# dguilliams3/book-recommendation-engine

Measured on AMD Instinct MI355X. Metric: exact top-10 queries/sec at 10M×1536 fp32 (1/8 GPU) + % HBM/MFMA roofline, higher is better.
Workload: dtype fp32

## Files before the change

book-recommendation-engine_amd/csrc/vs_api.hip:

```cpp
#include <algorithm>
#include <cstdio>
#include <cstring>
#include <mutex>
#include <shared_mutex>
#include <string>
#include <vector>

#include "../../include/vsearch.h"
#include "vs_internal.h"

using namespace vs;

constexpr int kI8FirstBackoff = 8;
constexpr int kI8MaxBackoff = 64;

struct vs_index {
  int d = 0;
  int metric = VS_METRIC_L2;
  int dtype = VS_DTYPE_F32;
  int device = 0;
  int esize = 4;
  int64_t ld = 0;
  int64_t ntotal = 0;
  int64_t capacity = 0;
// ... 652 lines not shown
    idx->rn2[p] = nullptr;
  }
  if (idx->fscale) (void)hipFree(idx->fscale);
  if (idx->anorm) (void)hipFree(idx->anorm);
  if (idx->anorm_b) (void)hipFree(idx->anorm_b);
  idx->anorm_b = nullptr;
  idx->codes = nullptr;
  idx->norms = nullptr;
  idx->fscale = nullptr;
  idx->anorm = nullptr;
  idx->capacity = 0;
}

struct SearchArgs {
  int mode = MODE_IP;
  const float* qbuf = nullptr;
  const void* qb16 = nullptr;
  const float* qaux = nullptr;
  const float* xaux = nullptr;
  int nq = 0, nq_pad = 0, k = 0;
  int64_t self0 = -1;
  float min_score = 0.0f;
  int raw = 0;
  bool l2_direct = false;
  bool host_wait = false;
  float* D = nullptr;
  int64_t* I = nullptr;
};

int run_topk(vs_index* idx, const SearchArgs& a, hipStream_t st, int force_engine);

int run_gemm(vs_index* idx, const SearchArgs& a, int need, hipStream_t st,
              const int* qlist = nullptr, const int* qcount = nullptr) {
  const int KP = kp_for(need);
  const int ntotal = (int)idx->ntotal;
  Scratch scr(st);
  Partials part;
  part.KP = KP;
  const int nqt = a.nq_pad / kBQ;
  const int ntiles = (ntotal + kBN - 1) / kBN;
  const int nsplit = qlist ? (int)std::max<int64_t>(1, std::min<int64_t>(ntiles, 256))
                           : (int)std::max<int64_t>(1, std::min<int64_t>(ntiles, (512 + nqt - 1) / nqt));
  part.P = 2 * nsplit;
  const size_t n = (size_t)a.nq_pad * part.P * KP;
  VS_HIP(scr.alloc((void**)&part.key, n * sizeof(float)), "vs: scratch");
  VS_HIP(scr.alloc((void**)&part.id, n * sizeof(int)), "vs: scratch");
  const void* qmat = a.qb16 ? a.qb16 : (const void*)a.qbuf;
  {
    KernelTimer tm(st, qlist ? nullptr : "gemm_topk");
    VS_HIP(launch_gemm_topk(KP, a.mode, idx->codes, a.xaux, qmat, a.qaux, idx->ld, idx->esize,
                            ntotal, a.nq_pad, nsplit, a.self0, part, st, qlist, qcount),
           "vs: gemm_topk launch");
    tm.stop();
  }
  VS_HIP(launch_merge_partials(a.mode, part, qlist ? a.nq_pad : a.nq, a.k, idx->id_base,
                               a.min_score, a.D, a.I, a.k, st, a.raw, qlist, qcount),
         "vs: merge launch");
  return VS_OK;
}

int adaptive_record(vs_index* idx, const int* handed, int n, hipStream_t st);
int run_paged(vs_index* idx, const SearchArgs& a, hipStream_t st, const int* gl = nullptr,
              const int* gc = nullptr);
int run_gemm_rescored(vs_index* idx, const SearchArgs& a, int need, int KF, int plane,
                      hipStream_t st, const int* gl, const int* gc);

static bool dump_enabled() {
  static const bool v = [] {
    const char* e = getenv("VS_X1_DUMP");
    return !e || atoi(e) != 0;
  }();
  return v;
}

static bool dump_mfma32() {
  const char* e = getenv("VS_X1_DUMP_MFMA");
  return e && atoi(e) == 32;
}

static int recut_mode() {
  const char* e = getenv("VS_X1_RECUT");
  const int v = e ? atoi(e) : 1;
  return v == 0 ? 0 : v == 2 ? 2 : 1;
}

constexpr int64_t kSmallFilterMinRows = 1 << 18;
bool small_filter_on() {
  const char* e = getenv("VS_SMALL_FILTER");
  return !e || atoi(e) != 0;
}
bool small_l2d_ok(int mode, const SearchArgs& a) {
  if (!(mode == MODE_L2 && a.l2_direct)) return true;
  const char* e = getenv("VS_SMALL_L2D");
  return !e || atoi(e) != 0;
}

bool skinny_deep_on() {
  const char* e = getenv("VS_SKINNY_DEEP");
  return !e || atoi(e) != 0;
}

static int x1_wg_target(int nqt) {
  const char* e = getenv("VS_X1_WGS");
  const int v = e ? atoi(e) : 0;
  return v > 0 ? v : nqt <= 8 ? 256 : 512;
}

static bool tail_wait_on(const SearchArgs& a, hipStream_t st) {
  const char* e = getenv("VS_TAIL_WAIT");
  if (e && atoi(e) == 0) return false;
  if (a.host_wait) return true;
  hipStreamCaptureStatus cs = hipStreamCaptureStatusNone;
  if (hipStreamIsCapturing(st, &cs) != hipSuccess) {
    (void)hipGetLastError();
    return false;
  }
  return cs == hipStreamCaptureStatusNone;
}

static int read_count(const int* dcount, hipStream_t st, int* out) {
  static thread_local int* pin = nullptr;
  if (!pin) VS_HIP(hipHostMalloc((void**)&pin, sizeof(int), hipHostMallocPortable), "vs: count");
  VS_HIP(hipMemcpyAsync(pin, dcount, sizeof(int), hipMemcpyDeviceToHost, st), "vs: count");
  VS_HIP(hipStreamSynchronize(st), "vs: count");
  *out = *pin;
  return VS_OK;
}

int run_filter_verify(vs_index* idx, const SearchArgs& a, int need, int KF, hipStream_t st,
                      int plane, bool last_plane, bool deep = false, const int* gl = nullptr,
                      const int* gc = nullptr) {
  const int ntotal = (int)idx->ntotal;
  const int mode = a.mode;
  const bool gathered = gl != nullptr;
  Scratch scr(st);
  X1Args x;
  x.nq_pad = (int)round_up(a.nq_pad, kX1Q);
  const int nq = gathered ? x.nq_pad : a.nq;
  const int nqt = x.nq_pad / kX1Q;
  const int ntiles = (ntotal + kX1Q - 1) / kX1Q;
  const int L = x1_lane_len();
  const int lists_per_cand = mode == MODE_IP && KF >= 64 ? 8 : 4;
  const int wg_target = x1_wg_target(nqt);
  x.nsplit = (int)std::max<int64_t>(
      std::min<int64_t>(ntiles, lists_per_cand * ((KF + L - 1) / L)),
      std::min<int64_t>(ntiles, (wg_target + nqt - 1) / nqt));
  if (deep)
    x.nsplit = (int)std::max<int64_t>(
        x.nsplit, std::min<int64_t>({ntiles, 512, (1ll << 30) / ((int64_t)x.nq_pad * 4 * 8 * 8)}));
  if (!gathered && !deep && plane == FILTER_BF16)
    x.nsplit = (int)std::min<int64_t>(ntiles, 2 * (int64_t)x.nsplit);
  const bool small = !gathered && !deep && a.nq <= skinny_plane_max_queries() && a.self0 < 0 &&
                     (mode == MODE_IP || (mode == MODE_L2 && idx->l2aug()));
  if (small) x.nsplit = (int)std::min<int64_t>(512, std::max<int64_t>(1, (ntiles + 3) / 4));
  x.nsplit = std::max(x.nsplit, 1);
  {
    static const int mult = [] {
      const char* e = getenv("VS_X1_SPLIT_MULT");
      return e && atoi(e) > 1 ? atoi(e) : 1;
    }();
    x.nsplit = (int)std::min<int64_t>(ntiles, (int64_t)x.nsplit * mult);
  }
  Partials part;
  part.KP = L;
  part.P = 4 * x.nsplit;
  const size_t np_ = (size_t)x.nq_pad * part.P * part.KP;
// ... 37 lines not shown
    if (i8) {
      float *sc = nullptr, *r = nullptr;
      VS_HIP(scr.alloc((void**)&sc, (size_t)qa_rows * sizeof(float)), "vs: scratch");
      VS_HIP(scr.alloc((void**)&r, (size_t)qa_rows * sizeof(float)), "vs: scratch");
      if (aug)
        VS_HIP(launch_quantize_i8_l2aug(Q, idx->ld, 0, qa_rows, idx->aug, nullptr, (int8_t*)qh, sc,
                                        r, nullptr, st),
               "vs: query plane");
      else
        VS_HIP(launch_quantize_i8(Q, idx->ld, 0, qa_rows, (int8_t*)qh, sc, r, st),
               "vs: query plane");
      qs = sc;
      qr2 = r;
    } else if (aug) {
      VS_HIP(launch_bf16_plane_l2aug(Q, idx->ld, 0, qa_rows, idx->aug, nullptr, (uint16_t*)qh,
                                     nullptr, nullptr, st),
             "vs: query plane");
    } else {
      VS_HIP(launch_bf16_plane(Q, idx->ld, 0, qa_rows, (uint16_t*)qh, st), "vs: query plane");
    }
    VS_HIP(launch_plane_zero_rows(qh, pb, qa_rows, x.nq_pad - qa_rows, st), "vs: query plane");
    QH = qh;
  }
  const unsigned* stats = idx->bstats[plane];
  x.filter = plane;
  x.XH = idx->fplane[plane];
  x.xs = idx->fscale;
  if (i8 && mode == MODE_COS) {
    float* cx = nullptr;
    VS_HIP(scr.alloc((void**)&cx, (size_t)idx->capacity * sizeof(float)), "vs: scratch");
    VS_HIP(launch_mul_arrays(idx->fscale, a.xaux, idx->capacity, cx, st), "vs: cosine factors");
    x.xs = cx;
    if (plane_rows) {
      qs = cx + a.self0;
    } else {
      float* cq = nullptr;
      VS_HIP(scr.alloc((void**)&cq, (size_t)qa_rows * sizeof(float)), "vs: scratch");
      VS_HIP(launch_mul_arrays(qs, qaux, qa_rows, cq, st), "vs: cosine factors");
      qs = cq;
    }
  }
  if (i8) {
    float* gm = nullptr;
    const size_t ng = (size_t)(idx->capacity / 16);
    VS_HIP(scr.alloc((void**)&gm, 2 * ng * sizeof(float)), "vs: scratch");
    VS_HIP(launch_group_max(x.xs, idx->capacity, gm, st, ntotal, gm + ng), "vs: factor bounds");
    x.xgmax = gm;
    x.xgmin = gm + ng;
  }
  x.xaux = a.xaux;
  x.QH = QH;
  x.qs = qs;
  x.qaux = qaux;
  x.nqa = qa_rows;
  x.ld = !aug ? idx->ld : i8 ? idx->ld + idx->aug_m : idx->ld + kAugBf16;
  x.ntotal = ntotal;
  x.self0 = self_rows ? a.self0 : -1;
  x.qrow = qrow;
  x.qcount = gc;
  const BoundArgs ba = aug ? make_bound_args_l2aug(idx->ld, idx->aug, plane)
                           : make_bound_args(idx->ld, plane);
  if (!gathered && !small && x1_dump_applies(kmode, plane) && dump_enabled() &&
      x1_pass_dumps(ntotal, x.nsplit)) {
    const int64_t lists = (int64_t)x.nq_pad * part.P;
    const int dR = (int)std::min<int64_t>(x1_dump_slots(), (int64_t(4) << 30) / (lists * 8));
    if (dR >= 16) {
      int *dc = nullptr, *ds = nullptr;
      hipError_t e = scr.alloc((void**)&dc, (size_t)lists * sizeof(int));
      if (e == hipSuccess) e = scr.alloc((void**)&ds, (size_t)lists * dR * 2 * sizeof(int));
      if (e == hipSuccess) {
        VS_HIP(scr.alloc((void**)&x.qcut, (size_t)qa_rows * sizeof(float)), "vs: scratch");
        double* bk = nullptr;
        VS_HIP(scr.alloc((void**)&bk, (size_t)qa_rows * sizeof(double)), "vs: scratch");
        VS_HIP(hipMemsetD32Async((hipDeviceptr_t)x.qcut, 0x7f7fffff, (size_t)qa_rows, st),
               "vs: cuts");
        VS_HIP(hipMemsetAsync(dc, 0, (size_t)lists * sizeof(int), st), "vs: dumps");
        VS_HIP(launch_qbound(mode, Q, idx->ld, qaux, plane, stats, qr2, qa_rows, bk, st, &ba),
               "vs: cuts");
        x.qbkey = bk;
        x.qcut_m = need;
        x.dump = true;
        x.dump32 = dump_mfma32();
        x.recut = recut_mode();
        x.dcount = dc;
        x.dslot = ds;
        x.dR = dR;
        x.dstats = device_stats(idx->device) ? device_stats(idx->device) + 6 : nullptr;
      } else {
        (void)hipGetLastError();
      }
    }
  }
  {
    KernelTimer whole(st, gathered ? nullptr : i8 ? "gemm_topk_x1_i8_pass" : "gemm_topk_x1_pass",
                      false);
    X1SpanTimer tm(i8 ? "gemm_topk_x1_i8" : "gemm_topk_x1",
                   i8 ? "gemm_topk_x1_i8_list" : "gemm_topk_x1_list");
    if (!gathered) x.timing = &tm;
    if (gathered && deep && !i8 && kmode == MODE_IP && a.self0 < 0 && skinny_deep_on()) {
      VS_HIP(launch_skinny_plane(FILTER_BF16, x.XH, x.QH, x.ld, ntotal, gc, nullptr, nullptr, part,
                                 st),
             "vs: skinny deep stage");
      x.qskip = skinny_plane_max_queries();
    }
    if (small) {
      int* cnt = nullptr;
      VS_HIP(scr.alloc((void**)&cnt, sizeof(int)), "vs: scratch");
      VS_HIP(hipMemsetD32Async((hipDeviceptr_t)cnt, a.nq, 1, st), "vs: count");
      KernelTimer ks(st, i8 ? "skinny_plane_topk_i8" : "skinny_plane_topk");
      VS_HIP(launch_skinny_plane(plane, x.XH, x.QH, x.ld, ntotal, cnt, qs, x.xs, part, st, a.nq),
             "vs: skinny first stage");
      ks.stop();
    } else {
      int nd = 0;
      VS_HIP(launch_gemm_topk_x1(kmode, x, part, st, &nd), "vs: gemm_topk_x1 launch");
    }
    x.timing = nullptr;
    whole.stop();
  }
  if (aug)
    VS_HIP(launch_l2aug_map(part.key, part.id, (int64_t)part.P * part.KP, qa_rows, qaux,
                            idx->aug.nref, x.qcut, st),
           "vs: L2 keys");

  float* Dk = nullptr;
  int64_t* Ik = nullptr;
  VS_HIP(scr.alloc((void**)&Dk, (size_t)nq * KF * sizeof(float)), "vs: scratch");
  VS_HIP(scr.alloc((void**)&Ik, (size_t)nq * KF * sizeof(int64_t)), "vs: scratch");
  if (KF > 64) {
    VS_HIP(launch_select_lists(part, L, nq, KF, Dk, Ik, st, gc), "vs: merge");
  } else if (select_heads_applies(part, L, KF)) {
    VS_HIP(launch_select_heads(part, nq, KF, Dk, Ik, st, gc), "vs: merge");
  } else {
    Partials mp = part;
    mp.KP = kp_for(KF);
    mp.KL = L;
    VS_HIP(launch_merge_partials(MODE_L2, mp, nq, KF, 0, 0.0f, Dk, Ik, KF, st, 0, nullptr, gc),
           "vs: merge");
  }
  Partials vp;
  vp.KP = kp_for(KF);
  vp.P = 1;
  int* flags = nullptr;
  int* qlist = nullptr;
  int* qcount = nullptr;
  VS_HIP(scr.alloc((void**)&vp.key, (size_t)nq * vp.KP * sizeof(float)), "vs: scratch");
  VS_HIP(scr.alloc((void**)&vp.id, (size_t)nq * vp.KP * sizeof(int)), "vs: scratch");
  VS_HIP(scr.alloc((void**)&flags, (size_t)nq * sizeof(int)), "vs: scratch");
  VS_HIP(scr.alloc((void**)&qlist, (size_t)x.nq_pad * sizeof(int)), "vs: scratch");
  VS_HIP(scr.alloc((void**)&qcount, 2 * sizeof(int)), "vs: scratch");
  const float* qinv = mode == MODE_COS ? qaux : nullptr;
  const float* xinv = mode == MODE_COS ? a.xaux : nullptr;
  VS_HIP(launch_verify_rescore(vmode, nq, KF, need, Dk, Ik, idx->codes, idx->norms, Q, qaux,
                               idx->ld, ba, stats, part, L, vp.key, vp.id, vp.KP, flags, st, qinv,
                               xinv, qr2, gc, x.qcut, idx->esize),
         "vs: verify");
  unsigned long long* dst = device_stats(idx->device);
  if (!dst) return fail(VS_E_HIP, "vs: statistics buffer");
  VS_HIP(launch_compact_flags(flags, nq, qlist, qcount, dst + 1, gathered ? nullptr : dst + 0, st),
         "vs: flags");
  if (wide_enabled())
    VS_HIP(launch_verify_wide(vmode, nq, qlist, qcount, KF, need, idx->codes, idx->norms, Q, qaux,
                              idx->ld, ba, stats, part, L, vp.key, vp.id, vp.KP, flags, st, qinv,
                              xinv, qr2, Dk, Ik, dst + 4, x.qcut, idx->esize),
           "vs: verify wide");
  VS_HIP(launch_compact_flags(flags, nq, qlist, qcount + 1, last_plane ? dst + 2 : dst + 3,
// ... 1306 lines not shown
```

book-recommendation-engine_amd/csrc/vs_gemm_x1.hip:

```cpp
#include <algorithm>
#include <climits>
#include <cmath>
#include <cstdlib>
#include <type_traits>

#include "vs_device.h"

#ifndef VS_X1_PROBE
#define VS_X1_PROBE 0
#endif
#define VS_X1_P(bit) ((VS_X1_PROBE & (bit)) != 0)

namespace vs {

#ifndef VS_X1_STAMP
#define VS_X1_STAMP 0
#endif
constexpr int kStampSeg = 9;
constexpr int kStampCnt = 3;
constexpr int kStampN = 2 * (kStampSeg + kStampCnt) + 2;
__device__ unsigned long long g_x1_stamps[kStampN];

namespace {

// ... 996 lines not shown
        pkey[o + e] = FLT_MAX;
        pid[o + e] = -1;
      }
    }
  }
}

template <int KR, int EL>
__global__ __launch_bounds__(256) void x1_replay_kernel(
    int* __restrict__ dcount, const int* __restrict__ dslot, float* __restrict__ pkey,
    int* __restrict__ pid, int P, int KP, int nqa, const float* __restrict__ qs,
    const float* __restrict__ xs, int64_t self0, int ntotal, int dR, int64_t nl,
    float* __restrict__ qcut, unsigned long long* __restrict__ stats) {
  const int64_t i = (int64_t)blockIdx.x * 256 + threadIdx.x;
  const int cnt = i < (int64_t)nqa * P ? dcount[i] : 0;
  {
    unsigned long long a = (unsigned long long)cnt, b = cnt > dR ? 1ull : 0ull;
    for (int o = 32; o > 0; o >>= 1) {
      a += __shfl_xor(a, o);
      b += __shfl_xor(b, o);
    }
    if ((threadIdx.x & 63) == 0 && a && stats) {
      atomicAdd(stats, a);
      if (b) atomicAdd(stats + 1, b);
    }
  }
  if (cnt == 0) return;
  dcount[i] = 0;
  const int q = (int)(i / P);
  if (cnt > dR) {
    qcut[q] = -FLT_MAX;
    return;
  }
  const float cut = qcut[q];
  const float qsc = EL == FILTER_I8 ? qs[q] : 0.0f;
  const int selfrow = self0 >= 0 ? (int)(self0 + q) : -1;
  static_assert(KR % 4 == 0, "lane lists move as 16-B pieces");
  float lk[KR];
  int li[KR];
  const int64_t o = i * KP;
#pragma unroll
  for (int e = 0; e < KR; e += 4) {
    const f32x4 kv = *(const f32x4*)(pkey + o + e);
    const int4 iv = *(const int4*)(pid + o + e);
    lk[e] = kv.x, lk[e + 1] = kv.y, lk[e + 2] = kv.z, lk[e + 3] = kv.w;
    li[e] = iv.x, li[e + 1] = iv.y, li[e + 2] = iv.z, li[e + 3] = iv.w;
  }
  const i32x2* sl = (const i32x2*)dslot + i;
  constexpr int kB = 8;
  for (int c0 = 0; c0 < cnt; c0 += kB) {
    i32x2 e[kB];
    float fx[kB];
#pragma unroll
    for (int j = 0; j < kB; ++j) e[j] = c0 + j < cnt ? sl[(int64_t)(c0 + j) * nl] : i32x2{-1, 0};
#pragma unroll
    for (int j = 0; j < kB; ++j)
      fx[j] = EL == FILTER_I8 && e[j][0] >= 0 && e[j][0] < ntotal ? xs[e[j][0]] : 0.0f;
#pragma unroll
    for (int j = 0; j < kB; ++j) {
      const int row = e[j][0];
      if (!(row >= 0 && row < ntotal && row != selfrow)) continue;
      const float key = x1_key<EL>(e[j][1], qsc, fx[j]);
      if (key < fminf(lk[KR - 1], cut)) list_insert<KR, int>(lk, li, key, row);
    }
  }
#pragma unroll
  for (int e = 0; e < KR; e += 4) {
    *(f32x4*)(pkey + o + e) = f32x4{lk[e], lk[e + 1], lk[e + 2], lk[e + 3]};
    *(int4*)(pid + o + e) = make_int4(li[e], li[e + 1], li[e + 2], li[e + 3]);
  }
}

static int x1_qg() {
  static const int v = [] {
    const char* e = getenv("VS_X1_QG");
    const int q = e ? atoi(e) : 0;
    return q > 0 ? q : 4;
  }();
  return v;
}

static hipError_t launch_qcut(const X1Args& a, Partials part, hipStream_t st);
static hipError_t launch_x1_replay_cut(const X1Args& a, Partials part, hipStream_t st);

static bool x1_group_rounds() {
  const char* e = getenv("VS_X1_XCDG");
  return !e || atoi(e) != 0;
}

constexpr int kHybMinTiles = 16;
constexpr int kX1SplitDen = 8;
static bool x1_hybrid_on() {
  const char* e = getenv("VS_X1_HYB");
  return e && atoi(e) != 0;
}

constexpr int kX1ShortChunkTiles = 40;
static int x1_chunk_tiles(int per_block, bool can_dump) {
  const char* e = getenv("VS_X1_CHUNK_TILES");
  const int v = e ? atoi(e) : 0;
  if (v > 0) return v;
  return can_dump && per_block >= 128 && per_block <= 3 * kX1ChunkTiles ? kX1ShortChunkTiles
                                                                        : kX1ChunkTiles;
}

static int x1_split_den() {
  const char* e = getenv("VS_X1_SPLIT");
  return e ? std::max(0, atoi(e)) : kX1SplitDen;
}
static bool x1_split_segments(int den) {
  const char* e = getenv("VS_X1_SPLITSEG");
  return e && atoi(e) != 0 && den >= 4 && (den & (den - 1)) == 0;
}
constexpr int kSplitMinTiles = 16;
static int x1_first_den(int el) {
  const char* e = getenv("VS_X1_QUARTER");
  if (!e) return el == FILTER_BF16 ? 4 : 0;
  const int v = atoi(e);
  return v == 1 ? 4 : v >= 2 ? v : 0;
}

template <int KR, int MODE, int EL>
static hipError_t x1_launch(const X1Args& a, Partials part, hipStream_t st, int* ndispatch) {
  const int ntiles = (a.ntotal + kT - 1) / kT;
  const int nqt = a.nq_pad / kT;
  const int per_block = (ntiles + a.nsplit - 1) / a.nsplit;
  const int qg = a.qcount ? nqt : x1_qg() * (x1_group_rounds() ? 1 : -1);
  const bool dump = a.dump && x1_has_dump(MODE, EL) && !a.qcount && a.qcut && a.qbkey &&
                    a.qcut_m > 0 && a.dcount && a.dslot && a.dR > 0;
  const int chunk_tiles = x1_chunk_tiles(per_block, dump);
  int nchunk = a.qcount ? 1 : std::max(1, (per_block + chunk_tiles - 1) / chunk_tiles);
  const int den = x1_split_den();
  const bool split = dump && nchunk < 4 && den >= 2 && per_block >= kSplitMinTiles;
  const bool cutting = dump && (nchunk >= 4 || split);
  const int tiles0 = (per_block + nchunk - 1) / nchunk;
  const bool hyb = dump && !split && x1_hybrid_on() && tiles0 >= kHybMinTiles;
  const bool later_dump = cutting || hyb;
  const int F = x1_first_den(EL);
  const bool quarter = cutting && !split && nchunk >= 4 && F >= 2 && per_block / (F * nchunk) >= 2;
  const bool sseg = split && x1_split_segments(den);
  int lg = 0;
  while ((1 << lg) < den) ++lg;
  const int nparts = split ? den : quarter ? F * nchunk : nchunk;
  const int nlaunch = sseg ? lg + 1 : split ? 2 : quarter ? nchunk + 1 : nchunk;
  const int64_t ldb = a.ld * filter_bytes(EL);
  if (a.qtile0 < 0) return hipErrorInvalidValue;
  for (int c = 0; c < nlaunch; ++c) {
    const int p0 = sseg    ? (c == 0 ? 0 : 1 << (c - 1))
                   : split   ? (c == 0 ? 0 : 1)
                   : quarter ? (c == 0 ? 0 : c == 1 ? 1 : F * (c - 1))
                             : c;
    const int p1 = sseg    ? (c == 0 ? 1 : 1 << c)
                   : split   ? (c == 0 ? 1 : den)
                   : quarter ? (c == 0 ? 1 : F * c)
                             : c + 1;
    if (a.timing)
      a.timing->begin(st, !(later_dump && nlaunch > 1) || c > 0, (double)(p1 - p0) / nparts);
    if (later_dump && c > 0 && x1_has_s16(MODE, EL) && !a.dump32) {
      if constexpr (x1_has_s16(MODE, EL))
        hipLaunchKernelGGL((gemm_topk_x1<KR, MODE, true, EL, false, true>), dim3(nqt * a.nsplit),
                           dim3(512), 0, st, (const char*)a.XH, a.xs, a.xaux, (const char*)a.QH,
                           a.qs, a.qaux, a.nqa, (int)(ldb / 64), a.ntotal, ntiles, a.nsplit, nqt,
                           a.qtile0, a.self0, a.qrow, a.qcount, p0, p1, nparts, part.KP, qg,
                           part.key, part.id, a.xgmax, a.xgmin, a.qcut, a.dcount, a.dslot, a.dR,
                           a.qskip);
    } else if (later_dump && c > 0) {
      if constexpr (x1_has_dump(MODE, EL))
        hipLaunchKernelGGL((gemm_topk_x1<KR, MODE, true, EL>), dim3(nqt * a.nsplit), dim3(512), 0,
                           st, (const char*)a.XH, a.xs, a.xaux, (const char*)a.QH, a.qs, a.qaux,
                           a.nqa, (int)(ldb / 64), a.ntotal, ntiles, a.nsplit, nqt, a.qtile0,
                           a.self0, a.qrow, a.qcount, p0, p1, nparts, part.KP, qg, part.key,
                           part.id, a.xgmax, a.xgmin, a.qcut, a.dcount, a.dslot, a.dR, a.qskip);
    } else if (hyb) {
      if constexpr (x1_has_dump(MODE, EL))
        hipLaunchKernelGGL((gemm_topk_x1<KR, MODE, false, EL, true>), dim3(nqt * a.nsplit),
                           dim3(512), 0, st, (const char*)a.XH, a.xs, a.xaux, (const char*)a.QH,
                           a.qs, a.qaux, a.nqa, (int)(ldb / 64), a.ntotal, ntiles, a.nsplit, nqt,
                           a.qtile0, a.self0, a.qrow, a.qcount, p0, p1, nparts, part.KP, qg,
                           part.key, part.id, a.xgmax, a.xgmin, a.qcut, a.dcount, a.dslot, a.dR, a.qskip);
    } else {
      hipLaunchKernelGGL((gemm_topk_x1<KR, MODE, false, EL>), dim3(nqt * a.nsplit), dim3(512), 0,
                         st, (const char*)a.XH, a.xs, a.xaux, (const char*)a.QH, a.qs, a.qaux,
                         a.nqa, (int)(ldb / 64), a.ntotal, ntiles, a.nsplit, nqt, a.qtile0,
                         a.self0, a.qrow, a.qcount, p0, p1, nparts, part.KP, qg, part.key,
                         part.id, a.xgmax, a.xgmin, nullptr, nullptr, nullptr, 0, a.qskip);
    }
    if (a.timing) a.timing->end(st);
    hipError_t e = hipGetLastError();
    if (e != hipSuccess) return e;
    if (hyb && c == 0) {
      e = launch_x1_replay(a, part, st);
      if (e != hipSuccess) return e;
    }
    if (cutting && c == 0) {
      e = launch_qcut(a, part, st);
      if (e != hipSuccess) return e;
    }
    if (later_dump && c > 0 && (sseg || ((c + 1) & c) == 0 || c + 1 == nlaunch)) {
      e = cutting && a.recut && c + 1 < nlaunch ? launch_x1_replay_cut(a, part, st)
                                                : launch_x1_replay(a, part, st);
      if (e != hipSuccess) return e;
    }
  }
  if (ndispatch) *ndispatch = nlaunch;
  return hipSuccess;
}

int x1_lane_len() { return 8; }
int x1_dump_slots() { return kDumpMaxR; }
bool x1_pass_dumps(int ntotal, int nsplit) {
  const int ntiles = (ntotal + kT - 1) / kT;
  const int per_block = (ntiles + nsplit - 1) / nsplit;
  const int ct = x1_chunk_tiles(per_block, true);
  const int nchunk = (per_block + ct - 1) / ct;
  return nchunk >= 4 || (x1_split_den() >= 2 && per_block >= kSplitMinTiles) ||
         (x1_hybrid_on() && (per_block + nchunk - 1) / nchunk >= kHybMinTiles);
}

hipError_t x1_stamps(unsigned long long* out, int reset) {
  hipError_t e = hipMemcpyFromSymbol(out, HIP_SYMBOL(g_x1_stamps), sizeof(g_x1_stamps));
  if (e == hipSuccess && reset) {
    unsigned long long z[kStampN] = {};
    e = hipMemcpyToSymbol(HIP_SYMBOL(g_x1_stamps), z, sizeof(z));
  }
  return e;
}

template <int EL>
static hipError_t x1_dispatch(int mode, const X1Args& a, Partials part, hipStream_t st,
                              int* ndispatch) {
  switch (mode) {
    case MODE_IP:
      return x1_launch<8, MODE_IP, EL>(a, part, st, ndispatch);
    case MODE_L2:
      if constexpr (EL == FILTER_I8) return hipErrorInvalidValue;
      else return x1_launch<8, MODE_L2, EL>(a, part, st, ndispatch);
    case MODE_COS:
      return x1_launch<8, MODE_COS, EL>(a, part, st, ndispatch);
    default:
      return hipErrorInvalidValue;
  }
}

hipError_t launch_gemm_topk_x1(int mode, const X1Args& a, Partials part, hipStream_t st,
                               int* ndispatch) {
  if (a.nq_pad % kT != 0 || a.ld % 64 != 0 || a.ld <= 0 || part.KP < x1_lane_len() ||
      part.P != 4 * a.nsplit || a.nsplit < 1 || a.ntotal <= 0)
    return hipErrorInvalidValue;
  if (a.filter == FILTER_I8) {
    if (!a.xs || !a.qs || !a.xgmax || !a.xgmin || a.ld > kI8MaxLd) return hipErrorInvalidValue;
    return x1_dispatch<FILTER_I8>(mode, a, part, st, ndispatch);
  }
  return x1_dispatch<FILTER_BF16>(mode, a, part, st, ndispatch);
}

bool x1_dump_applies(int mode, int filter) {
  return x1_has_dump(mode, filter) && (mode != MODE_COS || x1_cos_dump_on());
}

hipError_t launch_x1_replay(const X1Args& a, Partials part, hipStream_t st) {
  unsigned long long* stats = a.dstats;
  if (!a.dump || !a.dcount || a.nqa <= 0) return hipSuccess;
  if (part.KP < x1_lane_len() || part.KP % 4 != 0) return hipErrorInvalidValue;
  const int64_t n = (int64_t)a.nqa * part.P;
  const dim3 grid((unsigned)((n + 255) / 256));
  const int64_t nl = (int64_t)a.nq_pad * part.P;
  if (a.filter == FILTER_I8)
    hipLaunchKernelGGL((x1_replay_kernel<8, FILTER_I8>), grid, dim3(256), 0, st, a.dcount, a.dslot,
                       part.key, part.id, part.P, part.KP, a.nqa, a.qs, a.xs, a.self0, a.ntotal,
                       a.dR, nl, a.qcut, stats);
  else
    hipLaunchKernelGGL((x1_replay_kernel<8, FILTER_BF16>), grid, dim3(256), 0, st, a.dcount,
                       a.dslot, part.key, part.id, part.P, part.KP, a.nqa, a.qs, a.xs, a.self0,
                       a.ntotal, a.dR, nl, a.qcut, stats);
  return hipGetLastError();
}

int x1_list_len(int need) {
  return need + 8 <= 24   ? 24
         : need + 8 <= 32 ? 32
         : need + 8 <= 64 ? 64
         : need < 128 ? 128
         : need < 256 ? 256
// ... 1282 lines not shown
  if (qcount && q >= *qcount) return;
  const int64_t base = (int64_t)q * P * 8;
  for (int p = tid; p < P; p += 256) {
    hk[p] = lkey[base + (int64_t)p * 8];
    hi[p] = lid[base + (int64_t)p * 8];
  }
  if (tid == 0) {
    cnt = 0;
    ui = -1;
    uk = FLT_MAX;
  }
  __syncthreads();
  for (int p = tid; p < P; p += 256) {
    const float k0 = hk[p];
    const int i0 = hi[p];
    if (i0 < 0) continue;
    int r = 0;
    for (int t = 0; t < P; ++t) r += hi[t] >= 0 && lex_less(hk[t], hi[t], k0, i0) ? 1 : 0;
    if (r == KF - 1) {
      uk = k0;
      ui = i0;
    }
  }
  __syncthreads();
  const float U = uk;
  const int Ui = ui;
  for (int p = tid; p < P; p += 256) {
    if (Ui >= 0 && lex_less(U, Ui, hk[p], hi[p])) continue;
    const f32x4* kp = (const f32x4*)(lkey + base + (int64_t)p * 8);
    const int4* ip = (const int4*)(lid + base + (int64_t)p * 8);
    const f32x4 ka = kp[0], kb = kp[1];
    const int4 ia = ip[0], ib = ip[1];
    const float kk[8] = {ka.x, ka.y, ka.z, ka.w, kb.x, kb.y, kb.z, kb.w};
    const int ii[8] = {ia.x, ia.y, ia.z, ia.w, ib.x, ib.y, ib.z, ib.w};
#pragma unroll
    for (int j = 0; j < 8; ++j) {
      if (ii[j] < 0 || (Ui >= 0 && lex_less(U, Ui, kk[j], ii[j]))) break;
      const int s = atomicAdd(&cnt, 1);
      if (s < 8 * kHeadsMaxKF) {
        ck[s] = kk[j];
        ci[s] = ii[j];
      }
    }
  }
  __syncthreads();
  const int n = min(cnt, 8 * kHeadsMaxKF);
  float* dk = Dk + (int64_t)q * KF;
  int64_t* ik = Ik + (int64_t)q * KF;
  for (int j = tid; j < n; j += 256) {
    const float k0 = ck[j];
    const int i0 = ci[j];
    int r = 0;
    for (int t = 0; t < n; ++t) r += lex_less(ck[t], ci[t], k0, i0) ? 1 : 0;
    if (r < KF) {
      dk[r] = k0;
      ik[r] = i0;
    }
  }
  for (int j = n + tid; j < KF; j += 256) {
    dk[j] = FLT_MAX;
    ik[j] = -1;
  }
}

bool select_heads_applies(const Partials& part, int L, int KF) {
  const char* e = getenv("VS_SELECT_HEADS");
  if (e && atoi(e) == 0) return false;
  return L == 8 && part.KP == 8 && KF >= 1 && KF <= kHeadsMaxKF && part.P >= KF &&
         part.P <= kHeadsMaxP;
}

hipError_t launch_select_heads(Partials part, int nq, int KF, float* Dk, int64_t* Ik,
                               hipStream_t st, const int* qcount) {
  if (!select_heads_applies(part, 8, KF)) return hipErrorInvalidValue;
  if (nq <= 0) return hipSuccess;
  hipLaunchKernelGGL(select_heads_kernel, dim3(nq), dim3(256), 0, st, part.key, part.id, part.P,
                     KF, Dk, Ik, qcount);
  return hipGetLastError();
}

constexpr int kQcutThreads = 256;
__global__ __launch_bounds__(kQcutThreads) void qcut_kernel(
    const float* __restrict__ lkey, const int* __restrict__ lid, int P, int LKP, int L, int M,
    const double* __restrict__ bkey, int nq, float* __restrict__ cut) {
  const int q = blockIdx.x;
  const int tid = threadIdx.x;
  if (q >= nq) return;
  const int64_t base = (int64_t)q * P * LKP;
  const int n = P * L;
  constexpr int kR = 16;
  uint64_t v[kR];
  const bool regs = n <= kQcutThreads * kR;
  auto image = [&](int j) -> uint64_t {
    const int64_t o = base + (int64_t)(j / L) * LKP + j % L;
    return lid[o] >= 0 ? (uint64_t)key_order(lkey[o]) : (1ull << 32);
  };
#pragma unroll
  for (int i = 0; i < kR; ++i) {
    const int j = tid + kQcutThreads * i;
    v[i] = regs && j < n ? image(j) : (1ull << 32);
  }
  __shared__ int part[kQcutThreads / 64];
  auto count_below = [&](uint64_t y) {
    int c = 0;
    if (regs) {
#pragma unroll
      for (int i = 0; i < kR; ++i) c += v[i] < y ? 1 : 0;
    } else {
      for (int j = tid; j < n; j += kQcutThreads) c += image(j) < y ? 1 : 0;
    }
    for (int o = 32; o > 0; o >>= 1) c += __shfl_xor(c, o);
    __syncthreads();
    if ((tid & 63) == 0) part[tid >> 6] = c;
    __syncthreads();
    int t = 0;
#pragma unroll
    for (int w = 0; w < kQcutThreads / 64; ++w) t += part[w];
    return t;
  };
  if (count_below(1ull << 32) < M) return;
  uint64_t x = 0;
  for (int b = 31; b >= 0; --b)
    if (count_below(x + (1ull << b)) < M) x += 1ull << b;
  const float aM = key_unorder((uint32_t)x);
  const double tp = (double)aM + 2.000001 * bkey[q];
  if (tid == 0 && isfinite(tp) && tp < (double)FLT_MAX) {
    float t = (float)tp;
    if ((double)t < tp) t = nextafterf(t, INFINITY);
    if (t < cut[q]) cut[q] = t;
  }
}

template <int KR, int EL>
__global__ __launch_bounds__(256) void x1_replay_cut_kernel(
    int* __restrict__ dcount, const int* __restrict__ dslot, float* __restrict__ pkey,
    int* __restrict__ pid, int P, int KP, const float* __restrict__ qs,
    const float* __restrict__ xs, int64_t self0, int ntotal, int dR, int64_t nl,
    float* __restrict__ qcut, unsigned long long* __restrict__ stats, int M,
    const double* __restrict__ bkey) {
  __shared__ int hist[256];
  __shared__ int wsum[4];
  __shared__ int s_over, sel_digit, sel_before;
  const int q = blockIdx.x;
  const int tid = threadIdx.x, lane = tid & 63, wv = tid >> 6;
  const int nth = blockDim.x, nwv = nth >> 6;
  const bool has = tid < P;
  const int64_t i = (int64_t)q * P + tid;
  const int cnt = has ? dcount[i] : 0;
  {
    unsigned long long a = (unsigned long long)cnt, b = cnt > dR ? 1ull : 0ull;
    for (int o = 32; o > 0; o >>= 1) {
      a += __shfl_xor(a, o);
      b += __shfl_xor(b, o);
    }
    if (lane == 0 && a && stats) {
      atomicAdd(stats, a);
      if (b) atomicAdd(stats + 1, b);
    }
  }
  if (tid == 0) s_over = 0;
  const float cut = qcut[q];
  static_assert(KR % 4 == 0, "lane lists move as 16-B pieces");
  float lk[KR];
  int li[KR];
  const int64_t o = i * KP;
#pragma unroll
  for (int e = 0; e < KR; ++e) lk[e] = FLT_MAX, li[e] = -1;
  if (has) {
#pragma unroll
    for (int e = 0; e < KR; e += 4) {
      const f32x4 kv = *(const f32x4*)(pkey + o + e);
      const int4 iv = *(const int4*)(pid + o + e);
      lk[e] = kv.x, lk[e + 1] = kv.y, lk[e + 2] = kv.z, lk[e + 3] = kv.w;
      li[e] = iv.x, li[e + 1] = iv.y, li[e + 2] = iv.z, li[e + 3] = iv.w;
    }
  }
  __syncthreads();
  if (cnt > 0) {
    dcount[i] = 0;
    if (cnt > dR) {
      s_over = 1;
    } else {
      const float qsc = EL == FILTER_I8 ? qs[q] : 0.0f;
      const int selfrow = self0 >= 0 ? (int)(self0 + q) : -1;
      const i32x2* sl = (const i32x2*)dslot + i;
      constexpr int kB = 8;
      for (int c0 = 0; c0 < cnt; c0 += kB) {
        i32x2 e[kB];
        float fx[kB];
#pragma unroll
        for (int j = 0; j < kB; ++j)
          e[j] = c0 + j < cnt ? sl[(int64_t)(c0 + j) * nl] : i32x2{-1, 0};
#pragma unroll
        for (int j = 0; j < kB; ++j)
          fx[j] = EL == FILTER_I8 && e[j][0] >= 0 && e[j][0] < ntotal ? xs[e[j][0]] : 0.0f;
#pragma unroll
        for (int j = 0; j < kB; ++j) {
          const int row = e[j][0];
          if (!(row >= 0 && row < ntotal && row != selfrow)) continue;
          const float key = x1_key<EL>(e[j][1], qsc, fx[j]);
          if (key < fminf(lk[KR - 1], cut)) list_insert<KR, int>(lk, li, key, row);
        }
      }
#pragma unroll
      for (int e = 0; e < KR; e += 4) {
        *(f32x4*)(pkey + o + e) = f32x4{lk[e], lk[e + 1], lk[e + 2], lk[e + 3]};
        *(int4*)(pid + o + e) = make_int4(li[e], li[e + 1], li[e + 2], li[e + 3]);
      }
    }
  }
  __syncthreads();
  if (s_over) {
    if (tid == 0) qcut[q] = -FLT_MAX;
    return;
  }
  if (cut == -FLT_MAX) return;
  uint32_t v[KR];
  int nv = 0;
#pragma unroll
  for (int e = 0; e < KR; ++e) {
    v[e] = key_order(lk[e]);
    nv += li[e] >= 0 ? 1 : 0;
  }
  for (int o2 = 32; o2 > 0; o2 >>= 1) nv += __shfl_xor(nv, o2);
  if (lane == 0) wsum[wv] = nv;
  __syncthreads();
  int total = 0;
  for (int w2 = 0; w2 < nwv; ++w2) total += wsum[w2];
  if (total < M) return;
  uint32_t pre = 0;
  int want = M;
  for (int sh = 24; sh >= 0; sh -= 8) {
    for (int b = tid; b < 256; b += nth) hist[b] = 0;
    __syncthreads();
#pragma unroll
    for (int e = 0; e < KR; ++e)
      if (li[e] >= 0 && (sh == 24 || (v[e] >> (sh + 8)) == (pre >> (sh + 8))))
        atomicAdd(&hist[(v[e] >> sh) & 0xFF], 1);
    __syncthreads();
    if (wv == 0) {
      const int h0 = hist[4 * lane], h1 = hist[4 * lane + 1], h2 = hist[4 * lane + 2],
                h3 = hist[4 * lane + 3];
      const int own = h0 + h1 + h2 + h3;
      int inc = own;
      for (int o2 = 1; o2 < 64; o2 <<= 1) {
        const int t = __shfl_up(inc, o2);
        if (lane >= o2) inc += t;
      }
      const int before = inc - own;
      if (before < want && want <= inc) {
        int c = before, d = 4 * lane;
        const int hh[4] = {h0, h1, h2, h3};
        for (int e = 0; e < 4; ++e) {
          if (c + hh[e] >= want) {
            d = 4 * lane + e;
            break;
          }
          c += hh[e];
        }
        sel_digit = d;
        sel_before = c;
      }
    }
    __syncthreads();
    pre |= (uint32_t)sel_digit << sh;
    want -= sel_before;
  }
  if (tid == 0) {
    const float aM = key_unorder(pre);
    const double tp = (double)aM + 2.000001 * bkey[q];
    if (isfinite(tp) && tp < (double)FLT_MAX) {
      float t = (float)tp;
      if ((double)t < tp) t = nextafterf(t, INFINITY);
      if (t < cut) qcut[q] = t;
    }
  }
}

constexpr int kReplayCutMaxP = 256;

hipError_t launch_qbound(int mode, const float* Q, int64_t ld, const float* qn, int filter,
                         const unsigned* stats, const float* qr2i8, int nq, double* bkey,
                         hipStream_t st, const BoundArgs* bap) {
  if (nq <= 0) return hipSuccess;
  if (ld % 4 != 0) return hipErrorInvalidValue;
  const BoundArgs ba = bap ? *bap : make_bound_args(ld, filter);
#define VS_QB(MD) \
  hipLaunchKernelGGL(qbound_kernel<MD>, dim3(nq), dim3(64), 0, st, Q, ld, qn, ba, stats, qr2i8, nq, bkey)
  if (mode == MODE_IP)
    VS_QB(MODE_IP);
  else if (mode == MODE_L2)
    VS_QB(MODE_L2);
  else if (mode == MODE_COS)
    VS_QB(MODE_COS);
  else
    return hipErrorInvalidValue;
#undef VS_QB
  return hipGetLastError();
}

static hipError_t launch_qcut(const X1Args& a, Partials part, hipStream_t st) {
  const int nq = a.nqa;
  hipLaunchKernelGGL(qcut_kernel, dim3(nq), dim3(kQcutThreads), 0, st, part.key, part.id, part.P, part.KP,
                     x1_lane_len(), a.qcut_m, a.qbkey, nq, a.qcut);
  return hipGetLastError();
}

static hipError_t launch_x1_replay_cut(const X1Args& a, Partials part, hipStream_t st) {
  if (!a.dump || !a.dcount || a.nqa <= 0) return hipSuccess;
  if (part.KP < x1_lane_len() || part.KP % 4 != 0) return hipErrorInvalidValue;
  if (a.recut == 2 || part.P > kReplayCutMaxP) {
    const hipError_t e = launch_x1_replay(a, part, st);
    return e != hipSuccess ? e : launch_qcut(a, part, st);
  }
  const int64_t nl = (int64_t)a.nq_pad * part.P;
  const dim3 block((unsigned)((part.P + 63) / 64 * 64));
  if (a.filter == FILTER_I8)
    hipLaunchKernelGGL((x1_replay_cut_kernel<8, FILTER_I8>), dim3(a.nqa), block, 0, st, a.dcount,
                       a.dslot, part.key, part.id, part.P, part.KP, a.qs, a.xs, a.self0, a.ntotal,
                       a.dR, nl, a.qcut, a.dstats, a.qcut_m, a.qbkey);
  else
    hipLaunchKernelGGL((x1_replay_cut_kernel<8, FILTER_BF16>), dim3(a.nqa), block, 0, st, a.dcount,
                       a.dslot, part.key, part.id, part.P, part.KP, a.qs, a.xs, a.self0, a.ntotal,
                       a.dR, nl, a.qcut, a.dstats, a.qcut_m, a.qbkey);
  return hipGetLastError();
}


BoundArgs make_bound_args(int64_t ld, int filter) {
  BoundArgs ba;
  ba.filter = filter;
  const double u = std::ldexp(1.0, -23);
  const double n = (double)ld + 1.0;
  ba.gam = filter == FILTER_I8 ? 6.0 * std::ldexp(1.0, -24) : n * u / (1.0 - n * u);
  ba.norm_inf = 2.0 * (n * u / (1.0 - n * u));
  return ba;
}

BoundArgs make_bound_args_l2aug(int64_t ld, const L2Aug& g, int filter) {
  const bool i8 = filter == FILTER_I8;
  BoundArgs ba = make_bound_args(ld + (i8 ? g.m : kAugBf16), filter);
  ba.l2aug = 1;
  const double c = i8 ? (double)g.C : (double)g.Cb;
  ba.aug_q2 = (i8 ? (double)g.m : (double)kAugBf16) * c * c;
  ba.aug_nref = (double)g.nref;
  return ba;
}

}
```

book-recommendation-engine_amd/csrc/vs_internal.h:

```cpp
#pragma once

#include <hip/hip_runtime.h>

#include <cfloat>
#include <climits>
#include <cstdint>

namespace vs {

enum Mode : int { MODE_IP = 0, MODE_L2 = 1, MODE_COS = 2, MODE_L2D = 3 };

constexpr int kBN = 128;
constexpr int kBQ = 128;
constexpr int kBK = 32;
constexpr int kRowPad = 256;
constexpr int kGemvMaxQ = 8;
constexpr int kBlasThreshold = 20;
constexpr int kSkinnyMaxQ = 32;

__host__ __device__ inline uint16_t f32_to_bf16_rne(float f) {
  uint32_t u;
  __builtin_memcpy(&u, &f, 4);
  if ((u & 0x7F800000u) == 0x7F800000u && (u & 0x007FFFFFu))
    return (uint16_t)((u >> 16) | 0x0040u);
  u += 0x7FFFu + ((u >> 16) & 1u);
  return (uint16_t)(u >> 16);
}

struct Partials {
  float* key = nullptr;
  int* id = nullptr;
  int P = 0;
  int KP = 0;
  int KL = 0;
};

hipError_t launch_gemm_topk(int KP, int mode, const void* X, const float* xaux, const void* Q,
                            const float* qaux, int64_t ld, int esize, int ntotal, int nq_pad,
                            int nsplit, int64_t self0, Partials part, hipStream_t st,
                            const int* qlist = nullptr, const int* qcount = nullptr,
                            const float* fkey = nullptr, const int* fid = nullptr);
hipError_t launch_gemv_topk(int KP, int mode, int nq, const void* X, int esize, const float* Q,
                            int64_t ld, int ntotal, int nblocks, Partials part, hipStream_t st,
                            const float* fkey = nullptr, const int* fid = nullptr,
                            const int* run = nullptr);
hipError_t launch_skinny_plane(int filter, const void* XH, const void* QH, int64_t ld, int ntotal,
                               const int* qcount, const float* qs, const float* xs, Partials part,
                               hipStream_t st, int nq_hint = 0);
int skinny_plane_max_queries();
hipError_t launch_skinny_topk(int KP, int mode, int nq, const void* X, int esize,
                              const float* xaux, const void* Q, const float* qaux, int64_t ld,
                              int ntotal, int nblocks, Partials part, hipStream_t st,
                              const int* qcount = nullptr);
enum Filter : int { FILTER_BF16 = 0, FILTER_I8 = 1 };
inline int filter_bytes(int filter) { return filter == FILTER_I8 ? 1 : 2; }
__host__ __device__ inline int64_t plane_offset(int64_t row, int64_t byte, int64_t ldb) {
  return ((row >> 8) * (ldb >> 6) + (byte >> 6)) * 16384 + (row & 255) * 64 + (byte & 63);
}
struct X1Timing {
  virtual void begin(hipStream_t st, bool dominant, double share) = 0;
  virtual void end(hipStream_t st) = 0;
  virtual ~X1Timing() = default;
};
struct X1Args {
  X1Timing* timing = nullptr;
  int qskip = 0;
  int filter = FILTER_BF16;
  const void* XH = nullptr;
  const float* xs = nullptr;
  const float* xgmax = nullptr;
  const float* xgmin = nullptr;
  bool dump = false;
  bool dump32 = false;
  float* qcut = nullptr;
  const double* qbkey = nullptr;
  int qcut_m = 0;
  int recut = 1;
  int* dcount = nullptr;
  int* dslot = nullptr;
  int dR = 0;
  unsigned long long* dstats = nullptr;
  const float* xaux = nullptr;
  const void* QH = nullptr;
  int qtile0 = 0;
  const float* qs = nullptr;
  const float* qaux = nullptr;
  int nqa = 0;
  int64_t ld = 0;
  int ntotal = 0;
  int nq_pad = 0;
  int nsplit = 1;
  int64_t self0 = -1;
  const int* qrow = nullptr;
  const int* qcount = nullptr;
};
constexpr int kX1Q = 256;
constexpr int64_t kI8MaxLd = 131072;
int x1_list_len(int need);
int x1_lane_len();
hipError_t x1_stamps(unsigned long long* out, int reset);
hipError_t launch_gemm_topk_x1(int mode, const X1Args& a, Partials part, hipStream_t st,
                               int* ndispatch);
struct BoundArgs {
  int filter = FILTER_BF16;
  double gam = 0.0;
  double norm_inf = 0.0;
  int l2aug = 0;
  double aug_q2 = 0.0;
  double aug_nref = 0.0;
  int rows_exact = 0;
};
BoundArgs make_bound_args(int64_t ld, int filter);
struct L2Aug {
  int m = 0;
  float C = 0.0f;
  float nref = 0.0f;
  float Cb = 0.0f;
};
constexpr int kAugBf16 = 64;
BoundArgs make_bound_args_l2aug(int64_t ld, const L2Aug& g, int filter = FILTER_I8);
hipError_t launch_bound_stats(const float* norms, const float* rn2, int64_t n, unsigned* out,
                              hipStream_t st, bool accumulate = false);
hipError_t launch_resid_norms(const float* X, int64_t ld, int64_t r0, int64_t n, float* out,
                              hipStream_t st);
hipError_t launch_quantize_i8(const void* X, int64_t ld, int64_t r0, int64_t n, int8_t* codes,
                              float* scale, float* rn2, hipStream_t st, int xesize = 4);
hipError_t launch_quantize_i8_l2aug(const float* X, int64_t ld, int64_t r0, int64_t n,
                                    const L2Aug& g, const float* norms, int8_t* codes,
                                    float* scale, float* rn2, float* anorm, hipStream_t st);
hipError_t launch_bf16_plane_l2aug(const float* X, int64_t ld, int64_t r0, int64_t n,
                                   const L2Aug& g, const float* norms, uint16_t* plane, float* rn2,
                                   float* anorm, hipStream_t st);
hipError_t l2aug_params(const float* X, int64_t ld, int64_t r0, int64_t n, const float* norms,
                        L2Aug* out, hipStream_t st);
hipError_t launch_l2aug_map(float* key, const int* id, int64_t per_query, int nq,
                            const float* qn, float nref, float* qcut, hipStream_t st);
hipError_t launch_gather_queries(const float* src, int64_t ld, const float* aux, const int* gl,
                                 const int* count, int nslot, int64_t self0, float* dst,
                                 float* daux, int* drow, hipStream_t st);
hipError_t launch_add_counts(const int* count, int n, unsigned long long* acc, hipStream_t st);
hipError_t launch_compose_list(const int* outer, const int* inner, const int* count, int n,
                               int* out, hipStream_t st);
hipError_t launch_window_count(const int* count, int w0, int cap, int* out, hipStream_t st);
hipError_t launch_group_max(const float* f, int64_t n, float* out, hipStream_t st,
                            int64_t nvalid = 0, float* outmin = nullptr);
hipError_t launch_mul_arrays(const float* a, const float* b, int64_t n, float* out,
                             hipStream_t st);
hipError_t launch_verify_rescore(int mode, int nq, int KF, int M, const float* Dk,
                                 const int64_t* Ik, const void* X, const float* xn,
                                 const float* Q, const float* qn, int64_t ld, const BoundArgs& ba,
                                 const unsigned* stats, Partials lists, int L, float* okey,
                                 int* oid, int KP, int* fail, hipStream_t st,
                                 const float* qinv, const float* xinv, const float* qsc,
                                 const int* qcount = nullptr, const float* qcut = nullptr,
                                 int xesize = 4);
hipError_t launch_compact_flags(const int* flags, int n, int* list, int* count,
                                unsigned long long* total, unsigned long long* total_n,
                                hipStream_t st);
constexpr int kWideCap = 4096;
constexpr int kVerifyMaxKF = 1024;
hipError_t launch_select_lists(Partials part, int L, int nq, int KF, float* Dk, int64_t* Ik,
                               hipStream_t st, const int* qcount = nullptr);
bool select_heads_applies(const Partials& part, int L, int KF);
hipError_t launch_select_heads(Partials part, int nq, int KF, float* Dk, int64_t* Ik,
                               hipStream_t st, const int* qcount = nullptr);

struct ScratchChunk {
  void* p = nullptr;
  size_t size = 0;
  int dev = 0;
  hipEvent_t ev = nullptr;
  hipStream_t st = nullptr;
};
hipError_t scratch_chunk_get(size_t bytes, hipStream_t st, ScratchChunk* out);
void scratch_chunk_put(const ScratchChunk& c, hipStream_t st);
void scratch_trim();
hipError_t launch_verify_wide(int mode, int nq_max, const int* qlist, const int* count, int KF,
                              int M, const void* X, const float* xn, const float* Q,
                              const float* qn, int64_t ld, const BoundArgs& ba,
// ... 73 lines not shown
```

Baseline: 85260.

## Tighten int8 IP cut with exact rescoring of candidates below approximate threshold

Adds an exact-cut kernel for the int8 inner-product path. After each qcut or replay-cut it gathers up to 64 candidate rows whose approximate key falls below the M-th approximate key, rescores them in fp32 against the original vectors, and merges them into a per-query exact top-M list. It then sets a tighter per-query cut using the exact M-th key plus a smaller error bound, so later chunks can dump fewer rows. The int8 path also now uses quarter-first launch scheduling, which adds launches and extra fp32 row reads per query in exchange for fewer rows surviving the filter.

Result: faster. 89060, median of 6 (+4.5%).

```diff
diff --git a/book-recommendation-engine_amd/csrc/vs_api.hip b/book-recommendation-engine_amd/csrc/vs_api.hip
--- a/book-recommendation-engine_amd/csrc/vs_api.hip
+++ b/book-recommendation-engine_amd/csrc/vs_api.hip
@@ -758,6 +758,11 @@
   const char* e = getenv("VS_X1_RECUT");
   const int v = e ? atoi(e) : 1;
   return v == 0 ? 0 : v == 2 ? 2 : 1;
+}
+
+static bool ecut_enabled() {
+  const char* e = getenv("VS_X1_ECUT");
+  return !e || atoi(e) != 0;
 }
 
 constexpr int64_t kSmallFilterMinRows = 1 << 18;
@@ -961,6 +966,21 @@
         x.dump = true;
         x.dump32 = dump_mfma32();
         x.recut = recut_mode();
+        if (i8 && mode == MODE_IP && idx->esize == 4 && need <= kEcutMaxM && ecut_enabled()) {
+          int* ci = nullptr;
+          VS_HIP(scr.alloc((void**)&x.qam, (size_t)qa_rows * sizeof(float)), "vs: scratch");
+          VS_HIP(scr.alloc((void**)&x.ecut_key, (size_t)qa_rows * kEcutMaxM * sizeof(float)),
+                 "vs: scratch");
+          VS_HIP(scr.alloc((void**)&ci, (size_t)qa_rows * kEcutMaxM * sizeof(int)), "vs: scratch");
+          VS_HIP(hipMemsetD32Async((hipDeviceptr_t)x.qam, 0x7f7fffff, (size_t)qa_rows, st),
+                 "vs: cuts");
+          VS_HIP(hipMemsetAsync(ci, 0xFF, (size_t)qa_rows * kEcutMaxM * sizeof(int), st),
+                 "vs: cuts");
+          x.ecut_id = ci;
+          x.ecut_x = (const float*)idx->codes;
+          x.ecut_q = Q;
+          x.ecut_ld = idx->ld;
+        }
         x.dcount = dc;
         x.dslot = ds;
         x.dR = dR;
diff --git a/book-recommendation-engine_amd/csrc/vs_gemm_x1.hip b/book-recommendation-engine_amd/csrc/vs_gemm_x1.hip
--- a/book-recommendation-engine_amd/csrc/vs_gemm_x1.hip
+++ b/book-recommendation-engine_amd/csrc/vs_gemm_x1.hip
@@ -1102,6 +1102,7 @@
 
 static hipError_t launch_qcut(const X1Args& a, Partials part, hipStream_t st);
 static hipError_t launch_x1_replay_cut(const X1Args& a, Partials part, hipStream_t st);
+static hipError_t launch_x1_ecut(const X1Args& a, Partials part, hipStream_t st);
 
 static bool x1_group_rounds() {
   const char* e = getenv("VS_X1_XCDG");
@@ -1133,9 +1134,9 @@
   return e && atoi(e) != 0 && den >= 4 && (den & (den - 1)) == 0;
 }
 constexpr int kSplitMinTiles = 16;
-static int x1_first_den(int el) {
+static int x1_first_den(int el, bool ecut) {
   const char* e = getenv("VS_X1_QUARTER");
-  if (!e) return el == FILTER_BF16 ? 4 : 0;
+  if (!e) return el == FILTER_BF16 || ecut ? 4 : 0;
   const int v = atoi(e);
   return v == 1 ? 4 : v >= 2 ? v : 0;
 }
@@ -1156,7 +1157,8 @@
   const int tiles0 = (per_block + nchunk - 1) / nchunk;
   const bool hyb = dump && !split && x1_hybrid_on() && tiles0 >= kHybMinTiles;
   const bool later_dump = cutting || hyb;
-  const int F = x1_first_den(EL);
+  const bool ecut = MODE == MODE_IP && EL == FILTER_I8 && a.ecut_x && a.qam;
+  const int F = x1_first_den(EL, ecut);
   const bool quarter = cutting && !split && nchunk >= 4 && F >= 2 && per_block / (F * nchunk) >= 2;
   const bool sseg = split && x1_split_segments(den);
   int lg = 0;
@@ -1214,11 +1216,13 @@
     }
     if (cutting && c == 0) {
       e = launch_qcut(a, part, st);
+      if (e == hipSuccess && ecut) e = launch_x1_ecut(a, part, st);
       if (e != hipSuccess) return e;
     }
     if (later_dump && c > 0 && (sseg || ((c + 1) & c) == 0 || c + 1 == nlaunch)) {
-      e = cutting && a.recut && c + 1 < nlaunch ? launch_x1_replay_cut(a, part, st)
-                                                : launch_x1_replay(a, part, st);
+      const bool again = cutting && a.recut && c + 1 < nlaunch;
+      e = again ? launch_x1_replay_cut(a, part, st) : launch_x1_replay(a, part, st);
+      if (e == hipSuccess && again && ecut) e = launch_x1_ecut(a, part, st);
       if (e != hipSuccess) return e;
     }
   }
@@ -2667,7 +2671,7 @@
 constexpr int kQcutThreads = 256;
 __global__ __launch_bounds__(kQcutThreads) void qcut_kernel(
     const float* __restrict__ lkey, const int* __restrict__ lid, int P, int LKP, int L, int M,
-    const double* __restrict__ bkey, int nq, float* __restrict__ cut) {
+    const double* __restrict__ bkey, int nq, float* __restrict__ cut, float* __restrict__ qam) {
   const int q = blockIdx.x;
   const int tid = threadIdx.x;
   if (q >= nq) return;
@@ -2708,6 +2712,7 @@
   for (int b = 31; b >= 0; --b)
     if (count_below(x + (1ull << b)) < M) x += 1ull << b;
   const float aM = key_unorder((uint32_t)x);
+  if (tid == 0 && qam) qam[q] = aM;
   const double tp = (double)aM + 2.000001 * bkey[q];
   if (tid == 0 && isfinite(tp) && tp < (double)FLT_MAX) {
     float t = (float)tp;
@@ -2722,7 +2727,7 @@
     int* __restrict__ pid, int P, int KP, const float* __restrict__ qs,
     const float* __restrict__ xs, int64_t self0, int ntotal, int dR, int64_t nl,
     float* __restrict__ qcut, unsigned long long* __restrict__ stats, int M,
-    const double* __restrict__ bkey) {
+    const double* __restrict__ bkey, float* __restrict__ qam) {
   __shared__ int hist[256];
   __shared__ int wsum[4];
   __shared__ int s_over, sel_digit, sel_before;
@@ -2853,6 +2858,7 @@
   }
   if (tid == 0) {
     const float aM = key_unorder(pre);
+    if (qam) qam[q] = aM;
     const double tp = (double)aM + 2.000001 * bkey[q];
     if (isfinite(tp) && tp < (double)FLT_MAX) {
       float t = (float)tp;
@@ -2863,6 +2869,145 @@
 }
 
 constexpr int kReplayCutMaxP = 256;
+
+constexpr int kEcutCand = 64;
+__global__ __launch_bounds__(256) void x1_ecut_kernel(
+    const float* __restrict__ lkey, const int* __restrict__ lid, int P, int LKP, int L, int M,
+    const double* __restrict__ bkey, const float* __restrict__ qam, const float* __restrict__ X,
+    const float* __restrict__ Q, int64_t ld, int ntotal, float* __restrict__ ckey,
+    int* __restrict__ cid, float* __restrict__ qcut) {
+  constexpr int kU = kEcutMaxM + kEcutCand;
+  __shared__ int cand[kEcutCand];
+  __shared__ float uk[kU];
+  __shared__ int ui[kU];
+  __shared__ int wsum[4];
+  __shared__ int un;
+  const int q = blockIdx.x;
+  const int tid = threadIdx.x, lane = tid & 63, wv = tid >> 6;
+  const float cut = qcut[q];
+  const float aM = qam[q];
+  float* ck = ckey + (int64_t)q * kEcutMaxM;
+  int* ci = cid + (int64_t)q * kEcutMaxM;
+  if (tid < kEcutMaxM) {
+    ui[tid] = ci[tid];
+    uk[tid] = ck[tid];
+  }
+  const float* qrow = Q + (int64_t)q * ld;
+  const bool pairs = ld <= 256 * kQV;
+  QSlice qsl;
+  if (pairs) load_qslice(qrow, ld, lane, qsl);
+  if (cut == -FLT_MAX || !(aM < FLT_MAX)) return;
+  const bool vec = L == 8 && LKP % 4 == 0;
+  int ncand = 0;
+  for (int p0 = 0; p0 < P && ncand < kEcutCand; p0 += 256) {
+    const int p = p0 + tid;
+    int ids[8];
+    float lk[8];
+    int c = 0;
+    const int64_t o = ((int64_t)q * P + p) * LKP;
+#pragma unroll
+    for (int e = 0; e < 8; ++e) ids[e] = -1, lk[e] = FLT_MAX;
+    if (p < P && vec) {
+#pragma unroll
+      for (int e = 0; e < 8; e += 4) {
+        const f32x4 kv = *(const f32x4*)(lkey + o + e);
+        const int4 iv = *(const int4*)(lid + o + e);
+        lk[e] = kv.x, lk[e + 1] = kv.y, lk[e + 2] = kv.z, lk[e + 3] = kv.w;
+        ids[e] = iv.x, ids[e + 1] = iv.y, ids[e + 2] = iv.z, ids[e + 3] = iv.w;
+      }
+    } else if (p < P) {
+#pragma unroll
+      for (int e = 0; e < 8; ++e)
+        if (e < L) ids[e] = lid[o + e], lk[e] = lkey[o + e];
+    }
+#pragma unroll
+    for (int e = 0; e < 8; ++e) {
+      if (ids[e] >= 0 && ids[e] < ntotal && lk[e] <= aM)
+        ++c;
+      else
+        ids[e] = -1;
+    }
+    int inc = c;
+    for (int o2 = 1; o2 < 64; o2 <<= 1) {
+      const int t = __shfl_up(inc, o2);
+      if (lane >= o2) inc += t;
+    }
+    __syncthreads();
+    if (lane == 63) wsum[wv] = inc;
+    __syncthreads();
+    int before = ncand + inc - c;
+    for (int w = 0; w < wv; ++w) before += wsum[w];
+#pragma unroll
+    for (int e = 0; e < 8; ++e)
+      if (ids[e] >= 0) {
+        if (before < kEcutCand) cand[before] = ids[e];
+        ++before;
+      }
+    ncand += wsum[0] + wsum[1] + wsum[2] + wsum[3];
+  }
+  ncand = min(ncand, kEcutCand);
+  __syncthreads();
+  int m0 = 0;
+  for (int t = 0; t < kEcutMaxM; ++t) m0 += ui[t] >= 0 ? 1 : 0;
+  if (tid == 0) un = m0;
+  __syncthreads();
+  if (tid < ncand) {
+    const int r = cand[tid];
+    bool found = false;
+    for (int t = 0; t < m0; ++t) found |= ui[t] == r;
+    if (!found) ui[atomicAdd(&un, 1)] = r;
+  }
+  __syncthreads();
+  const int n = un;
+  if (pairs) {
+    for (int j = m0 + 2 * wv; j < n; j += 8) {
+      const int ra = ui[j], rb = j + 1 < n ? ui[j + 1] : ra;
+      double da, db;
+      wave_dot2<false, float>(X + (int64_t)ra * ld, X + (int64_t)rb * ld, qsl, ld, lane, da, db);
+      if (lane == 0) {
+        uk[j] = exact_key<MODE_IP>((float)da, q, ra, nullptr, nullptr, nullptr, nullptr);
+        if (j + 1 < n)
+          uk[j + 1] = exact_key<MODE_IP>((float)db, q, rb, nullptr, nullptr, nullptr, nullptr);
+      }
+    }
+  } else {
+    for (int j = m0 + wv; j < n; j += 4) {
+      const int r = ui[j];
+      const double acc = wave_dot<false, float>(X + (int64_t)r * ld, qrow, ld, lane);
+      if (lane == 0) uk[j] = exact_key<MODE_IP>((float)acc, q, r, nullptr, nullptr, nullptr, nullptr);
+    }
+  }
+  __syncthreads();
+  if (tid < n) {
+    const float k0 = uk[tid];
+    const int i0 = ui[tid];
+    int rank = 0;
+    for (int t = 0; t < n; ++t) rank += lex_less(uk[t], ui[t], k0, i0) ? 1 : 0;
+    if (rank < M) {
+      ck[rank] = k0;
+      ci[rank] = i0;
+    }
+    if (rank == M - 1) {
+      const double tp = (double)k0 + 1.000001 * bkey[q];
+      if (isfinite(tp) && tp < (double)FLT_MAX) {
+        float t = (float)tp;
+        if ((double)t < tp) t = nextafterf(t, INFINITY);
+        if (t < cut) qcut[q] = t;
+      }
+    }
+  }
+}
+
+static hipError_t launch_x1_ecut(const X1Args& a, Partials part, hipStream_t st) {
+  if (!a.ecut_x || !a.ecut_q || !a.qam || !a.ecut_key || !a.ecut_id || a.nqa <= 0)
+    return hipSuccess;
+  if (a.qcut_m < 1 || a.qcut_m > kEcutMaxM || a.ecut_ld % 4 != 0 || x1_lane_len() > 8)
+    return hipErrorInvalidValue;
+  hipLaunchKernelGGL(x1_ecut_kernel, dim3(a.nqa), dim3(256), 0, st, part.key, part.id, part.P,
+                     part.KP, x1_lane_len(), a.qcut_m, a.qbkey, a.qam, a.ecut_x, a.ecut_q,
+                     a.ecut_ld, a.ntotal, a.ecut_key, a.ecut_id, a.qcut);
+  return hipGetLastError();
+}
 
 hipError_t launch_qbound(int mode, const float* Q, int64_t ld, const float* qn, int filter,
                          const unsigned* stats, const float* qr2i8, int nq, double* bkey,
@@ -2887,7 +3032,7 @@
 static hipError_t launch_qcut(const X1Args& a, Partials part, hipStream_t st) {
   const int nq = a.nqa;
   hipLaunchKernelGGL(qcut_kernel, dim3(nq), dim3(kQcutThreads), 0, st, part.key, part.id, part.P, part.KP,
-                     x1_lane_len(), a.qcut_m, a.qbkey, nq, a.qcut);
+                     x1_lane_len(), a.qcut_m, a.qbkey, nq, a.qcut, a.qam);
   return hipGetLastError();
 }
 
@@ -2903,11 +3048,11 @@
   if (a.filter == FILTER_I8)
     hipLaunchKernelGGL((x1_replay_cut_kernel<8, FILTER_I8>), dim3(a.nqa), block, 0, st, a.dcount,
                        a.dslot, part.key, part.id, part.P, part.KP, a.qs, a.xs, a.self0, a.ntotal,
-                       a.dR, nl, a.qcut, a.dstats, a.qcut_m, a.qbkey);
+                       a.dR, nl, a.qcut, a.dstats, a.qcut_m, a.qbkey, a.qam);
   else
     hipLaunchKernelGGL((x1_replay_cut_kernel<8, FILTER_BF16>), dim3(a.nqa), block, 0, st, a.dcount,
                        a.dslot, part.key, part.id, part.P, part.KP, a.qs, a.xs, a.self0, a.ntotal,
-                       a.dR, nl, a.qcut, a.dstats, a.qcut_m, a.qbkey);
+                       a.dR, nl, a.qcut, a.dstats, a.qcut_m, a.qbkey, a.qam);
   return hipGetLastError();
 }
 
diff --git a/book-recommendation-engine_amd/csrc/vs_internal.h b/book-recommendation-engine_amd/csrc/vs_internal.h
--- a/book-recommendation-engine_amd/csrc/vs_internal.h
+++ b/book-recommendation-engine_amd/csrc/vs_internal.h
@@ -76,6 +76,12 @@
   const double* qbkey = nullptr;
   int qcut_m = 0;
   int recut = 1;
+  const float* ecut_x = nullptr;
+  const float* ecut_q = nullptr;
+  int64_t ecut_ld = 0;
+  float* qam = nullptr;
+  float* ecut_key = nullptr;
+  int* ecut_id = nullptr;
   int* dcount = nullptr;
   int* dslot = nullptr;
   int dR = 0;
@@ -95,6 +101,7 @@
   const int* qcount = nullptr;
 };
 constexpr int kX1Q = 256;
+constexpr int kEcutMaxM = 32;
 constexpr int64_t kI8MaxLd = 131072;
 int x1_list_len(int need);
 int x1_lane_len();
```
